# artiom-matvei/RLAO

Hardware: AMD Instinct MI355X
Metric: AO env-steps/sec (batched loops) (higher is better)
Workload: dtype f32; 1 GPU; 8m / 20x20 Shack-Hartmann, 256 batched envs per GPU, integrator closed loop (BASELINE.json configs[1]); envs_per_gpu=256, envs_total=256, resolution=120, n_valid_act=357, n_signal=632, layers=1, controller=leaky integrator, gain 0.5, noise=photon, parallelism=env-shards x1, all-gather of episode returns

## Files before the change

### rlao_amd/csrc/common.hpp

```cpp
#pragma once
#include <hip/hip_runtime.h>
#include <stdint.h>
#include <stddef.h>

#include <string>
#include <vector>

#include "aoenv.h"

namespace ao {

constexpr int kWave = 64;
constexpr int kMaxLayer = 8;
constexpr int kMtN = 624;
constexpr int kMaxSplits = 16;
constexpr int kMaxModes = 512;

int fail(const char* fmt, ...);
#define AO_HIP(call)                                                                          \
    do {                                                                                      \
        hipError_t e_ = (call);                                                               \
        if (e_ != hipSuccess)                                                                 \
            return ::ao::fail("%s:%d: %s -> %s", __FILE__, __LINE__, #call, hipGetErrorString(e_)); \
    } while (0)
// ... 219 lines not shown
    T* ret;
    T* strehl;
    T* scal;
    T* total;
    T* residual;
    const double* part;
    int n_tiles, n_pupil, telemetry_index;
    int n_act, n_valid_act, do_integrate;
    T leak, gain_from_obs;
    double src_scale;
};
template <typename T>
int launch_recon_finish(const FinishArgs<T>& fa, int n_env, hipStream_t st);
template <typename T>
int launch_sh_tail(const T* frame, const T* wfs_max, const ShConst<T>& sc, T* signal, const T* fac_m,
                   const T* fac_m2c_t, int n_modes, const FinishArgs<T>& fa, int n_env, int R, int n_subap, int n_valid,
                   int max_group, hipStream_t st);
struct DetectorCfg {
    int active;
    int photon_noise, bits, emccd;
    float qe, dark_e, fwc, gain, readout_noise;
    uint32_t seed_lo, seed_hi;
    uint32_t frame_counter;
    uint32_t env_offset;
};

}
#include "poisson_alias.hpp"
namespace ao {

struct StepArgs {
    KArgs<float> k;
    ShConst<float> sc;
    FinishArgs<float> fa;
    float* frame;
    int store_phase, store_frame;
    float* signal;
    float* wfs_max;
    const float* fac_m;
    const float* fac_m2c_t;
    const short* slot_of;
    const float* amp_pupil;
    const float* gxa;
    const float* gya;
    DetectorCfg det;
    PoissonAlias pa;
    const float* ring_x[kMaxLayer];
    int ring_splits[kMaxLayer];
    const int* outer_idx;
    int n_outer;
    float* next_zx[kMaxLayer];
    int next_sx[kMaxLayer], next_sy[kMaxLayer];
    const int* inner_idx;
    int n_inner, zx_ld;
    int n_modes, n_subap, n_valid, n_env;
};
int step_fused_supported(int R, int n_subap, int n_valid, int n_act, int n_modes);
int step_alias_capacity(int n_act);
int launch_env_step(const StepArgs& a, hipStream_t st);

template <typename T>
struct RolloutActionArgs {
    const T* obs;
    T* action;
    const T* fr;
    const T* fl_t;
    const int* act_slot;
    const T* sigma_env;
    T gain, sigma;
    int n_act, n_valid_act, n_filter;
    uint32_t seed_lo, seed_hi, counter, env_offset;
};
constexpr size_t kRolloutLdsMax = 160 * 1024;
size_t rollout_action_lds(int n_valid_act, int n_filter, size_t esz);
template <typename T>
int launch_rollout_action(const RolloutActionArgs<T>& a, int n_env, hipStream_t st);

template <typename T>
struct DisturbArgs {
    const T* coefs;
    T* seen;
    const T* modes_t;
    const double* amp;
    const double* freq;
    const double* phase;
    int n_valid_act, n_modes, n_lines;
    int64_t tau;
};
template <typename T>
int launch_disturb_apply(const DisturbArgs<T>& a, int n_env, hipStream_t st);

template <typename T>
int launch_convert_from_f64(const double* src, T* dst, size_t n, hipStream_t st);

template <typename T> struct cx;
struct FftPlan {
    int n;
    int np;
    int n_fac;
    int fac[12];
    unsigned magic_ns[12];
    unsigned magic_m[12];
};
int make_fft_plan(int n, FftPlan* pl);
template <typename T>
struct PyrArgs {
// ... 50 lines not shown
```

### rlao_amd/csrc/env.hip

```cpp
#include <algorithm>
#include <cmath>
#include <cstdarg>
#include <cstdio>
#include <cstring>
#include <initializer_list>
#include <new>
#include <utility>

#include "common.hpp"
#include "detector.hpp"
#include "disturb.hpp"
#include "policy.hpp"
#include "sh_device.hpp"

namespace ao {

static thread_local std::string g_err;

int fail(const char* fmt, ...) {
    char buf[1024];
    va_list ap;
    va_start(ap, fmt);
    vsnprintf(buf, sizeof(buf), fmt, ap);
    va_end(ap);
    g_err = buf;
    return 1;
}

struct LayerClock {
    double ratio[2] = {0, 0};
    double buff[2] = {0, 0};
};

struct RingAhead { bool valid = false; int sx = 0, sy = 0, buf = 0; };

struct Layer {
    int N = 0, S = 0, nin = 0, nout = 0, K = 0;
    size_t scr_off = 0;
    void* ab = nullptr;
    int* inner_idx = nullptr;
    int* outer_idx = nullptr;
    bool have_ab = false, have_in = false, have_out = false;
    double weight = 0;
    LayerClock clk;
    int org[2] = {0, 0};
    uint32_t* mt_cur = nullptr;
    int* pos_cur = nullptr;
    uint32_t* mt_alt = nullptr;
    int* pos_alt = nullptr;
    int ring_pending = 0;
    const void* ring_src = nullptr;
    RingAhead ahead;
    bool gather_next = false;
    bool minmax_dirty = false;
    int env_rounds = 0;
};

}

using namespace ao;

struct AoEnv {
    AoCfg c{};
    int device = 0;
    size_t esz = 4;
    int R = 0, A = 0, nAct = 0, E = 0, L = 0, nSig = 0, nSub = 0, nVal = 0;
    int p = 0, n = 0, n_pupil = 0;
    Layer layer[kMaxLayer];
    size_t scr_elems = 0;
    int Kmax = 0, noutmax = 0, Smax = 0;
    bool uniform = true;
    int last_zx_layer = 0;
    bool per_env_wind = false;
    EnvClock* env_clk[2] = {nullptr, nullptr};
    int clk_cur = 0;
    int wind_pixels = 1;
    LayerTaps* env_taps = nullptr;
    bool per_env_r0 = false;
    std::vector<double> h_r0;
    double* xi_scale = nullptr;
    const double* sigma() const { return per_env_r0 ? xi_scale : nullptr; }
    bool use_coefs_img = false;
    bool defer_ring = true;
    bool have[AOENV_C_COUNT] = {false};
    double units = 1.0;
    void* screen = nullptr;
    void* minmax = nullptr;
    void* zx_pipe = nullptr;
    const void* last_zx = nullptr;
    bool use_lookahead = true;
    void* zx = nullptr;
    void* xbuf = nullptr;
    void* gx = nullptr;
    void* gy = nullptr;
    void* gxt = nullptr;
    void* modes = nullptr;
    void* dm_opd = nullptr;
    int* act_idx = nullptr;
    uint8_t* pupil = nullptr;
    void* opd_atm = nullptr;
    void* coefs = nullptr;
    void* dm_prev = nullptr;
    void* coefs_seen = nullptr;
    void* step_cmd = nullptr;
    void* cmd() const { return step_cmd ? step_cmd : coefs; }
    struct Disturb {
        bool set = false;
        int M = 0, J = 0;
        int64_t t0 = 0;
        void* modes_t = nullptr;
        double* par = nullptr;
        size_t modes_cap = 0, par_cap = 0;
    } disturb;
    float* dm_rows = nullptr;
    void* coefs_img = nullptr;
    void* phase = nullptr;
    void* scal = nullptr;
    double* part = nullptr;
    int n_tiles = 0;
    void* total = nullptr;
    void* residual = nullptr;
    void* wfs_max = nullptr;
    void* amp = nullptr;
    int* subap_idx = nullptr;
    uint8_t* valid2d = nullptr;
// ... 503 lines not shown
    fa.do_integrate = integrate;
    fa.leak = (T)env->c.leak;
    fa.gain_from_obs = (T)gain;
    fa.src_scale = 6.283185307179586476925286766559 / env->c.src_wavelength;
    return fa;
}

template <typename T>
int recon_product(AoEnv* env, int* splits, hipStream_t st) {
    const int Kp = (env->n_modes + 3) & ~3;
    if (env->n_modes > 0 && env->use_factored_recon && env->fac_m2c && env->tbuf &&
        (size_t)Kp * (env->nSig + env->A) < (size_t)env->A * env->nSig) {
        T* t = env->as<T>(env->tbuf);
        if constexpr (std::is_same<T, float>::value) {
            if (env->use_mfma) {
                const int s1 = gemm_splits(env->E, Kp, env->nSig);
                AO_TRY(launch_gemm_nt_mfma(env->as<float>(env->signal), env->as<float>(env->fac_m), t, env->E, Kp, env->nSig, env->nSig,
                                           env->nSig, s1, st));
                *splits = cdiv(env->A, 64) >= 32 ? 1 : gemm_splits(env->E, env->A, Kp);
                int xs = s1;
                if (s1 > 1 && cdiv(env->A, 64) >= 8) {
                    AO_TRY(launch_sum_slabs(t, (size_t)env->E * Kp, s1, st));
                    xs = 1;
                }
                return launch_gemm_nt_mfma(t, env->as<float>(env->fac_m2c), env->as<float>(env->vbuf), env->E, env->A, Kp, Kp, Kp, *splits,
                                           st, xs, (size_t)env->E * Kp);
            }
        }
        *splits = 1;
        AO_TRY(launch_gemm_nt<T>(env->as<T>(env->signal), env->as<T>(env->fac_m), t, env->E, Kp, env->nSig, env->nSig, env->nSig, Kp, st));
        return launch_gemm_nt<T>(t, env->as<T>(env->fac_m2c), env->as<T>(env->vbuf), env->E, env->A, Kp, Kp, Kp, env->A, st);
    }
    return gemm_dispatch<T>(env, env->as<T>(env->signal), env->as<T>(env->recon), env->as<T>(env->vbuf), env->E, env->A, env->nSig,
                            splits, st);
}

template <typename T>
int run_recon(AoEnv* env, const T* d_action, T* d_obs, T* d_reward, T* d_strehl, int telemetry_index, int integrate,
              double gain, hipStream_t st) {
    int splits = 1;
    {
        AO_PROF(env, GEMM_RECON, st);
        AO_TRY(recon_product<T>(env, &splits, st));
    }
    {
        FinishArgs<T> fa = finish_args<T>(env, d_action, d_obs, d_reward, d_strehl, telemetry_index, integrate, gain, splits);
        AO_PROF(env, RECON_FINISH, st);
        AO_TRY(launch_recon_finish<T>(fa, env->E, st));
    }
    if (integrate) AO_TRY(refresh_dense_dm<T>(env, st));
    return 0;
}

template <typename T>
bool fused_step_ok(const AoEnv*) { return false; }
template <>
bool fused_step_ok<float>(const AoEnv* env) {
    return env->use_fused_step && env->use_fast_wfs && env->use_mfma && env->use_fused_tail && env->c.wfs_type == AOENV_WFS_SH && env->c.dm_separable && env->n_modes > 0 &&
           env->c.max_group == 1 && env->L > 0 && env->uniform && env->c.cam_res == env->R && env->force_path == 0 &&
           step_fused_supported(env->R, env->nSub, env->nVal, env->nAct, env->n_modes) != 0;
}

template <typename T>
void fill_phase_args(AoEnv* env, PhaseArgs& pa, PhaseBuffers<T>& pb, int update_atm, int store_atm, int store_phase) {
    pa = PhaseArgs{};
    pa.n_layer = env->L;
    pa.S = env->layer[0].S;
    pa.foot = (env->layer[0].N / 2 - env->R / 2) + 1;
    pa.update_atm = (update_atm && env->L > 0 && !env->atm_user_defined) ? 1 : 0;
    pa.store_atm = store_atm;
    pa.store_phase = store_phase;
    for (int l = 0; l < env->L; ++l) {
        const Layer& y = env->layer[l];
        pa.S_l[l] = y.S;
        pa.foot_l[l] = (y.N / 2 - env->R / 2) + 1;
        pa.screen[l] = env->screen_ptr(l);
        pa.minmax[l] = env->minmax_ptr(l);
        pa.minmax_dirty[l] = y.minmax_dirty ? 1 : 0;
        LayerTaps& t = pa.taps[l];
        t.oy = y.org[0];
        t.ox = y.org[1];
        taps_from_buff(y.clk.buff, t);
        t.weight = y.weight;
    }
    pa.env_taps = env->per_env_wind ? env->env_taps : nullptr;
    pa.n_env = env->E;
    pb = PhaseBuffers<T>{};
    pb.opd_atm = env->as<T>(env->opd_atm);
    pb.coefs = env->as<T>(env->cmd());
    pb.coefs_img = env->use_coefs_img && env->coefs_img ? env->as<T>(env->coefs_img) : nullptr;
    pb.s1a = env->use_coefs_img && env->c.dm_separable ? env->dm_rows : nullptr;
    pb.dm_opd = env->c.dm_separable ? nullptr : env->as<T>(env->dm_opd);
    pb.gx = env->as<T>(env->gx);
    pb.gy = env->as<T>(env->gy);
    pb.gxt = env->as<T>(env->gxt);
    pb.gxa = env->gxa;
    pb.gya = env->gya;
    pb.ga_stride = env->ga_stride;
    pb.act_idx = env->act_idx;
    pb.pupil = env->pupil;
    pb.phase = env->as<T>(env->phase);
    pb.part = env->part;
    pb.wfs_max = env->as<T>(env->wfs_max);
}

template <typename T>
int run_fused_step(AoEnv*, int, const void*, void*, void*, void*, double, bool, hipStream_t) { return fail("fused step: float32 only"); }
template <>
int run_fused_step<float>(AoEnv* env, int i, const void* d_action, void* d_obs, void* d_reward, void* d_strehl, double gain,
                          bool observable, hipStream_t st) {
    if (env->amp_pupil_dirty) {
        const size_t R2 = (size_t)env->R * env->R;
        if (env->h_pupil.size() != R2 || env->h_amp.size() != R2) return fail("pupil / WFS amplitude have not been uploaded");
        std::vector<float> t(R2);
        for (size_t q = 0; q < R2; ++q) t[q] = env->h_pupil[q] ? (float)env->h_amp[q] : -1.f;
        AO_HIP(hipMemcpyAsync(env->amp_pupil, t.data(), R2 * sizeof(float), hipMemcpyHostToDevice, st));
        AO_HIP(hipStreamSynchronize(st));
        env->amp_pupil_dirty = false;
    }
    StepArgs a{};
    PhaseArgs pa;
    PhaseBuffers<float> pb;
    fill_phase_args<float>(env, pa, pb, 1, env->store_opd_atm ? 1 : 0, 1);
    a.k = make_phase_kargs<float>(pa, pb, env->R, env->nAct, env->A, env->c.atm_wavelength, env->c.src_wavelength);
    a.sc = sh_const<float>(env);
    a.fa = finish_args<float>(env, static_cast<const float*>(d_action), static_cast<float*>(d_obs),
                              static_cast<float*>(d_reward), static_cast<float*>(d_strehl), i, 1, gain, 1);
    a.fa.n_tiles = 1;
    a.frame = env->as<float>(env->frame);
    a.store_phase = a.store_frame = (observable || env->store_opd_atm) ? 1 : 0;
    a.signal = env->as<float>(env->signal);
    a.wfs_max = env->as<float>(env->wfs_max);
    a.fac_m = env->as<float>(env->fac_m);
    a.fac_m2c_t = env->as<float>(env->fac_m2c_t);
    a.slot_of = env->slot_of;
    a.amp_pupil = env->amp_pupil;
    a.gxa = env->gxa;
    a.gya = env->gya;
    if (env->det.active) env->det.frame_counter += 1;
    a.det = env->det;
    a.pa = env->alias();
    take_rings(env, a);
    const Layer& y0 = env->layer[0];
    a.outer_idx = y0.outer_idx;
    a.n_outer = y0.nout;
    a.inner_idx = y0.inner_idx;
    a.n_inner = y0.nin;
    a.zx_ld = y0.K;
    a.n_modes = env->n_modes;
    a.n_subap = env->nSub;
    a.n_valid = env->nVal;
    a.n_env = env->E;
    {
        AO_PROF(env, ENV_STEP, st);
        AO_TRY(launch_env_step(a, st));
    }
    rings_written(env);
    return 0;
}

struct SeenCommand {
    AoEnv* env;
    ~SeenCommand() { env->step_cmd = nullptr; }
};
template <typename T>
int apply_disturbance(AoEnv* env, int i, hipStream_t st) {
    const AoEnv::Disturb& d = env->disturb;
    const size_t n = (size_t)env->E * d.M * d.J;
    DisturbArgs<T> a{};
    a.coefs = env->as<T>(env->coefs);
    a.seen = env->as<T>(env->coefs_seen);
    a.modes_t = env->as<T>(d.modes_t);
    a.amp = d.par;
    a.freq = d.par + n;
    a.phase = d.par + 2 * n;
    a.n_valid_act = env->A;
    a.n_modes = d.M;
    a.n_lines = d.J;
    a.tau = d.t0 + (int64_t)i + 1;
    AO_TRY(launch_disturb_apply<T>(a, env->E, st));
    env->step_cmd = env->coefs_seen;
    return refresh_dense_dm<T>(env, st);
}

template <typename T>
int step_t(AoEnv* env, int i, const void* d_action, void* d_obs, void* d_frame, void* d_reward, void* d_strehl,
           double gain, bool observable, hipStream_t st) {
    const bool fused_step = fused_step_ok<T>(env);
    SeenCommand seen{env};
    if (env->disturb.set) AO_TRY(apply_disturbance<T>(env, i, st));
    AO_TRY(advance_atmosphere<T>(env, fused_step, st));
    env->atm_user_defined = false;
    if (fused_step) {
        AO_TRY(run_fused_step<T>(env, i, d_action, d_obs, d_reward, d_strehl, gain, observable, st));
        env->step_cmd = nullptr;
        if (d_frame)
            AO_HIP(hipMemcpyAsync(d_frame, env->frame, (size_t)env->E * env->c.cam_res * env->c.cam_res * sizeof(T),
                                  hipMemcpyDeviceToDevice, st));
        return 0;
// ... 30 lines not shown
        AO_TRY(run_recon<T>(env, static_cast<const T*>(d_action), static_cast<T*>(d_obs), static_cast<T*>(d_reward),
                            static_cast<T*>(d_strehl), i, 1, gain, st));
    }
    if (d_frame)
        AO_HIP(hipMemcpyAsync(d_frame, env->frame, (size_t)env->E * env->c.cam_res * env->c.cam_res * sizeof(T),
                              hipMemcpyDeviceToDevice, st));
    return 0;
}

struct BufInfo {
    void* ptr;
    size_t bytes;
};

int buf_info(AoEnv* env, int which, BufInfo* b) {
    const size_t z = env->esz, E = env->E, R2 = (size_t)env->R * env->R;
    switch (which) {
        case AOENV_B_SCREEN: *b = {nullptr, env->scr_elems * z}; return 0;
        case AOENV_B_OPD_ATM: *b = {env->opd_atm, E * R2 * z}; return 0;
        case AOENV_B_COEFS: *b = {env->coefs, E * env->A * z}; return 0;
        case AOENV_B_PHASE: *b = {env->phase, E * R2 * z}; return 0;
        case AOENV_B_FRAME: *b = {env->frame, E * (size_t)env->c.cam_res * env->c.cam_res * z}; return 0;
        case AOENV_B_SIGNAL: *b = {env->signal, E * env->nSig * z}; return 0;
        case AOENV_B_TOTAL: *b = {env->total, (size_t)env->c.n_loop * E * z}; return 0;
        case AOENV_B_RESIDUAL: *b = {env->residual, (size_t)env->c.n_loop * E * z}; return 0;
        case AOENV_B_WFS_MAX: *b = {env->wfs_max, E * z}; return 0;
        case AOENV_B_XI: *b = {env->last_zx ? const_cast<void*>(env->last_zx) : env->zx, E * env->layer[env->last_zx_layer].K * z}; return 0;
        case AOENV_B_MT_STATE: *b = {nullptr, (size_t)env->L * E * (kMtN + 1) * 4}; return 0;
        case AOENV_B_COUNTERS: *b = {nullptr, 16}; return 0;
        case AOENV_B_DM_PREV: *b = {env->dm_prev, E * env->A * z}; return 0;
        case AOENV_B_COEFS_SEEN: *b = {env->coefs_seen, E * env->A * z}; return 0;
        default: return fail("unknown buffer id %d", which);
    }
}

}

struct DeviceGuard {
    int prev = -1;
    bool ok = false;
    explicit DeviceGuard(int device) {
        if (hipGetDevice(&prev) != hipSuccess) prev = -1;
        ok = prev == device || hipSetDevice(device) == hipSuccess;
        if (prev == device) prev = -1;
    }
    ~DeviceGuard() { if (prev >= 0) (void)hipSetDevice(prev); }
    DeviceGuard(const DeviceGuard&) = delete;
    DeviceGuard& operator=(const DeviceGuard&) = delete;
};
#define AO_CHECK_ENV(env)                                                             \
    if (!(env)) return fail("null AoEnv");                                            \
    DeviceGuard ao_device_guard((env)->device);                                       \
    if (!ao_device_guard.ok) return fail("hipSetDevice(%d) failed", (env)->device)
static int upload_layer_table(AoEnv* env, int kind, int l, const void* h, size_t bytes) {
    if (l < 0 || l >= env->L) return fail("layer %d outside [0, %d)", l, env->L);
    Layer& y = env->layer[l];
    const int S = y.S, N = y.N;
    auto need = [&](size_t n) { return bytes == n ? 0 : fail("ring table %d of layer %d: got %zu bytes, expected %zu", kind, l, bytes, n); };
    if (kind == AOENV_C_AB) {
        AO_TRY(need((size_t)y.nout * y.K * 8));
        for (int j = 0; j < env->L; ++j) forget_lookahead(env->layer[j]);
        AO_TRY(upload_real(env, y.ab, static_cast<const double*>(h), (size_t)y.nout * y.K));
        y.have_ab = true;
        return 0;
    }
    if (kind != AOENV_C_INNER_IDX && kind != AOENV_C_OUTER_IDX) return fail("table %d is not a per-layer table", kind);
    const int cnt = kind == AOENV_C_INNER_IDX ? y.nin : y.nout;
    AO_TRY(need((size_t)cnt * 4));
    const int32_t* ix = static_cast<const int32_t*>(h);
    for (int i = 0; i < cnt; ++i)
        if (ix[i] < 0 || ix[i] >= S * S) return fail("ring index %d out of the %dx%d screen", ix[i], S, S);
    if (kind == AOENV_C_INNER_IDX)
        for (int i = 0; i < cnt; ++i) {
            const int r = ix[i] / S, c = ix[i] % S;
            if (r < 1 || r > N || c < 1 || c > N) return fail("inner ring index %d is not interior", ix[i]);
        }
    AO_HIP(hipMemcpy(kind == AOENV_C_INNER_IDX ? y.inner_idx : y.outer_idx, h, (size_t)cnt * 4, hipMemcpyHostToDevice));
    (kind == AOENV_C_INNER_IDX ? y.have_in : y.have_out) = true;
    return 0;
}

template <typename T>
int atm_update_t(AoEnv* env, hipStream_t st) {
    AO_TRY(advance_atmosphere<T>(env, false, st));
    env->atm_user_defined = false;
    return run_phase<T>(env, 1, 1, st);
}

#define AO_DISPATCH(env, fn, ...) ((env)->c.dtype == AOENV_F32 ? fn<float>(__VA_ARGS__) : fn<double>(__VA_ARGS__))

extern "C" {

const char* aoenv_last_error(void) { return g_err.c_str(); }
int aoenv_abi_version(void) { return AOENV_ABI_VERSION; }

int aoenv_create(const AoCfg* cfg, int device, AoEnv** out) {
    if (!cfg || !out) return fail("aoenv_create: null argument");
    if (cfg->abi_version != AOENV_ABI_VERSION) return fail("ABI version %d != %d", cfg->abi_version, AOENV_ABI_VERSION);
    if (cfg->dtype != AOENV_F32 && cfg->dtype != AOENV_F64) return fail("bad dtype %d", cfg->dtype);
    if (cfg->n_env < 1 || cfg->resolution < 2) return fail("bad n_env / resolution");
    if (cfg->n_layer < 0 || cfg->n_layer > kMaxLayer) return fail("n_layer %d out of range [0, %d]", cfg->n_layer, kMaxLayer);
    if (cfg->n_subap < 1 || cfg->resolution % cfg->n_subap) return fail("resolution %% n_subap != 0");
    if (cfg->n_layer > 0) {
        if (cfg->layer_res < cfg->resolution + 4) return fail("layer_res %d < R + 4", cfg->layer_res);
        if (cfg->n_inner != 8 * cfg->layer_res - 16 || cfg->n_outer != 4 * cfg->layer_res + 4)
            return fail("n_inner / n_outer do not match layer_res");
        for (int l = 0; l < cfg->n_layer; ++l)
            if (cfg->layer_res_l[l] != 0 && cfg->layer_res_l[l] < cfg->resolution + 4)
                return fail("layer_res_l[%d] = %d < R + 4", l, cfg->layer_res_l[l]);
    }
    if (cfg->n_signal != 2 * cfg->n_valid_subap) return fail("n_signal != 2 n_valid_subap");
    if (cfg->wfs_type != AOENV_WFS_SH && cfg->wfs_type != AOENV_WFS_PYRAMID) return fail("unknown wfs_type %d", cfg->wfs_type);
    if (cfg->wfs_type == AOENV_WFS_PYRAMID) {
        if (cfg->pyr_n_res < cfg->resolution || cfg->pyr_n_res % 2 || cfg->cam_res < 1 || cfg->pyr_n_res % cfg->cam_res)
            return fail("pyramid: nRes %d must be even, >= R and a multiple of the camera size %d", cfg->pyr_n_res, cfg->cam_res);
        if (cfg->pyr_n_theta < 1) return fail("pyramid: n_theta must be >= 1");
        if (cfg->pyr_q_lo < 0 || cfg->pyr_q_hi + cfg->n_subap > cfg->cam_res) return fail("pyramid: quadrants outside the camera");
    }
    if (cfg->max_group < 1) return fail("max_group must be >= 1");
    int ndev = 0;
    AO_HIP(hipGetDeviceCount(&ndev));
    if (device < 0 || device >= ndev) return fail("device %d not in [0, %d)", device, ndev);
    DeviceGuard ao_device_guard(device);
    if (!ao_device_guard.ok) return fail("hipSetDevice(%d) failed", device);

    AoEnv* e = new (std::nothrow) AoEnv();
    if (!e) return fail("out of host memory");
    e->c = *cfg;
    e->device = device;
    e->esz = cfg->dtype == AOENV_F32 ? 4 : 8;
    e->R = cfg->resolution; e->A = cfg->n_valid_act; e->nAct = cfg->n_act; e->E = cfg->n_env; e->L = cfg->n_layer;
    e->nSig = cfg->n_signal; e->nSub = cfg->n_subap; e->nVal = cfg->n_valid_subap;
    e->p = e->R / e->nSub; e->n = 2 * e->p;
    e->layer[0].N = cfg->layer_res;
    e->layer[0].S = cfg->layer_res + 2;
    for (int l = 0; l < e->L; ++l) {
        Layer& y = e->layer[l];
        y.N = cfg->layer_res_l[l] ? cfg->layer_res_l[l] : cfg->layer_res;
        y.S = y.N + 2;
        y.nin = 8 * y.N - 16;
        y.nout = 4 * y.N + 4;
        y.K = y.nin + y.nout;
        y.scr_off = e->scr_elems;
        e->scr_elems += (size_t)e->E * y.S * y.S;
        e->Kmax = std::max(e->Kmax, y.K);
        e->noutmax = std::max(e->noutmax, y.nout);
        e->Smax = std::max(e->Smax, y.S);
        if (y.N != e->layer[0].N) e->uniform = false;
    }
    const size_t z = e->esz, E = e->E, R2 = (size_t)e->R * e->R;
    int rc = 0;
    auto A_ = [&](void** p, size_t bytes) { if (!rc) rc = dmalloc(e, p, bytes); };
    if (e->L > 0) {
        A_(&e->screen, e->scr_elems * z);
        A_(&e->minmax, (size_t)e->L * E * 2 * z);
        if (cfg->dtype == AOENV_F32) {
            A_(&e->zx_pipe, (size_t)2 * e->L * E * e->Kmax * z);
        }
        A_(&e->zx, E * e->Kmax * z);
        A_(&e->xbuf, (size_t)e->L * kMaxSplits * E * e->noutmax * z);
        for (int l = 0; l < e->L; ++l) {
            Layer& y = e->layer[l];
            A_((void**)&y.mt_cur, E * kMtN * 4);
            A_((void**)&y.pos_cur, E * 4);
            A_((void**)&y.mt_alt, E * kMtN * 4);
            A_((void**)&y.pos_alt, E * 4);
            if (l > 0 && e->uniform) {
                y.ab = e->layer[0].ab;
                y.inner_idx = e->layer[0].inner_idx;
                y.outer_idx = e->layer[0].outer_idx;
                continue;
            }
            A_(&y.ab, (size_t)y.nout * y.K * z);
            A_((void**)&y.inner_idx, (size_t)y.nin * 4);
            A_((void**)&y.outer_idx, (size_t)y.nout * 4);
        }
    }
    A_(&e->gx, (size_t)e->R * e->nAct * z);
    A_(&e->gy, (size_t)e->R * e->nAct * z);
    A_(&e->gxt, (size_t)((e->nAct + 3) & ~3) * (size_t)(cdiv(e->R, 128) * 128) * z);
    if (!cfg->dm_separable) {
        A_(&e->modes, R2 * e->A * z);
        A_(&e->dm_opd, E * R2 * z);
    }
    A_((void**)&e->act_idx, (size_t)e->A * 4);
    A_((void**)&e->pupil, R2);
    A_(&e->opd_atm, E * R2 * z);
    A_(&e->coefs, E * e->A * z);
    A_(&e->coefs_seen, E * e->A * z);
    A_(&e->dm_prev, E * e->A * z);
    A_(&e->phase, E * R2 * z);
    A_(&e->scal, E * 4 * z);
    e->n_tiles = phase_tiles(e->R, e->nAct, e->esz);
    A_((void**)&e->part, E * (size_t)e->n_tiles * 4 * sizeof(double));
    A_(&e->total, (size_t)cfg->n_loop * E * z);
    A_(&e->residual, (size_t)cfg->n_loop * E * z);
    A_(&e->wfs_max, E * z);
    A_(&e->amp, R2 * z);
    A_((void**)&e->subap_idx, (size_t)e->nVal * 4);
    A_((void**)&e->valid2d, (size_t)e->nSub * e->nSub);
    A_((void**)&e->slot_of, (size_t)e->nSub * e->nSub * sizeof(short));
    A_((void**)&e->amp_pupil, R2 * sizeof(float));
    e->ga_stride = std::max(8, ((cdiv(e->nAct, 4) + 3) / 4) * 4);
    A_((void**)&e->gxa, (size_t)(cdiv(e->R, 128) * 128) * 4 * e->ga_stride * sizeof(float));
    A_((void**)&e->gya, (size_t)(cdiv(e->R, 128) * 128) * 4 * e->ga_stride * sizeof(float));
    if (e->A > 1024 && !rc) { rc = alloc_dm_rows(e); e->use_coefs_img = true; }
    A_(&e->sh_ref, (size_t)2 * e->nVal * z);
    A_(&e->tw, (size_t)e->n * 2 * z);
    A_(&e->phs, (size_t)e->p * 2 * z);
    A_(&e->frame, E * (size_t)cfg->cam_res * cfg->cam_res * z);
    A_(&e->signal, E * e->nSig * z);
    A_(&e->recon, (size_t)e->A * e->nSig * z);
    A_(&e->fac_m, (size_t)kMaxModes * e->nSig * z);
    A_(&e->fac_m2c_t, (size_t)kMaxModes * e->A * z);
    if (cfg->wfs_type == AOENV_WFS_PYRAMID) {
        const size_t N = cfg->pyr_n_res;
        e->pyr_chunk = cfg->pyr_n_theta < 4 ? cfg->pyr_n_theta : 4;
        A_(&e->pyr_mask, N * N * 2 * z);
        A_(&e->pyr_tt, (size_t)cfg->pyr_n_theta * R2 * z);
        A_(&e->pyr_tw, N * 2 * z);
        A_(&e->pyr_t1, E * e->pyr_chunk * (size_t)e->R * N * 2 * z);
        A_(&e->pyr_t2, E * e->pyr_chunk * N * N * 2 * z);
    }
    A_(&e->vbuf, (size_t)kMaxSplits * E * e->A * z);
    {
        const PoissonAliasHost& ph = poisson_alias_host();
        int budget = (int)ph.tab.size();
        if (cfg->wfs_type == AOENV_WFS_SH && e->p == fast6::P && e->R <= 128 && e->nAct <= 32) budget = std::min(budget, step_alias_capacity(e->nAct));
        ph.prefix(budget, &e->alias_words, &e->alias_lmax);
// ... 1390 lines not shown
```

### rlao_amd/csrc/step_kernel.hip

```cpp
#include "common.hpp"

#include "sh_device.hpp"
#include "detector.hpp"
#include "ring_device.hpp"

#include "camera_sh6.hpp"


namespace ao {

typedef float f32x4s __attribute__((ext_vector_type(4)));

template <typename P>
__device__ inline float ld_or0(const P* __restrict__ p, long idx, bool ok) {
    const float v = (float)p[ok ? idx : 0];
    return ok ? v : 0.f;
}

namespace fstep {
constexpr int TX = 128, PR = 64;
constexpr int WR = 16 + 3, WC = 32 + 4;
constexpr int WC4 = WC / 4;
constexpr int NV4 = (WR * WC4 + 63) / 64;
}

struct StepLds {
    int cimg, s1, mapt, slot, e0, sl, img, total;
    int tab, tab_cap;
};

static StepLds step_lds_layout(int n_act, int n_subap, int n_valid, int n_modes) {
    using namespace fstep;
    StepLds L;
    const int nAp = (n_act + 3) & ~3, SS = nAp + 1;
    int o = 0;
    auto take = [&](int words) { const int at = o; o += (words + 3) & ~3; return at; };
    const int sl_words = (2 * n_valid + 3) & ~3, img_words = n_act * n_act + n_modes;
    L.cimg = take(n_act * n_act);
    L.s1 = take(2 * PR * SS);
    L.mapt = take(16 * WR * WC);
    L.tab = L.cimg;
    L.tab_cap = o - L.tab;
    L.slot = take((n_subap * n_subap + 1) / 2);
    L.e0 = take(std::max(2 * n_valid * fast6::EST, sl_words + img_words));
    L.sl = L.e0;
    L.img = L.e0 + sl_words;
    L.total = o;
    return L;
}

template <bool PE>
__device__ inline const LayerTaps& step_taps(const PhaseArgs& pa, int l, int e) {
    if constexpr (PE) return pa.env_taps[(size_t)l * pa.n_env + e];
    else return pa.taps[l];
}

template <int KS, bool PE>
__global__ void __launch_bounds__(1024) k_env_step_sh6(const StepArgs a, const StepLds L) {
    using namespace fstep;
    using fast6::EST;
    extern __shared__ __align__(16) unsigned char lds_raw[];
    float* lds = reinterpret_cast<float*>(lds_raw);
    const KArgs<float>& k = a.k;
    const int R = k.R, nA = k.n_act, S = k.pa.S;
    const int nAp = (nA + 3) & ~3, SS = nAp + 1;
    float* cimg = lds + L.cimg;
    float* s1 = lds + L.s1;
    const int w_ = threadIdx.x >> 6;
    float* mapt = lds + L.mapt + w_ * (WR * WC);
    short* slot_s = reinterpret_cast<short*>(lds + L.slot);
    cplx<float>* E0 = reinterpret_cast<cplx<float>*>(lds + L.e0);
    float* sl = lds + L.sl;
    float* img_s = lds + L.img;
    const uint32_t* tab_s = reinterpret_cast<const uint32_t*>(lds + L.tab);
    __shared__ double red[4][16];
    __shared__ double red_tail[16];
    __shared__ float red_mx[16];

    const int e = blockIdx.x;
    const int tid = threadIdx.x, w = tid >> 6, lane = tid & 63;
    const int lc = lane & 15, lq = lane >> 4;
    const int band = w >> 2, cg = w & 3;
    const size_t pix0 = (size_t)e * R * R;
    const int n_sub = a.n_subap, n_valid = a.n_valid;

    const float ctab = fast6::cos_table_lane<float>();
    f32x4s gx_raw[2][2], gy_raw[2];
#pragma unroll
    for (int tt = 0; tt < 2; ++tt) {
        const f32x4s* src = reinterpret_cast<const f32x4s*>(a.gxa) + (2 * cg + tt) * 2 * 64 + (tid & 63);
        gx_raw[tt][0] = src[0];
        gx_raw[tt][1] = src[64];
    }
    const int rt = w >> 1, ct = w & 1;
    {
        const f32x4s* src = reinterpret_cast<const f32x4s*>(a.gya) + rt * 2 * 64 + (tid & 63);
        gy_raw[0] = src[0];
        gy_raw[1] = src[64];
    }
    float mm_pre[kMaxLayer];
#pragma unroll
    for (int l = 0; l < kMaxLayer; ++l)
        mm_pre[l] = l < k.pa.n_layer ? static_cast<const float*>(k.pa.minmax[l])[2 * e + (tid & 1)] : 0.f;
    const bool has_act = tid < k.n_valid_act;
    const int act_px = k.pb.act_idx[has_act ? tid : 0];
    const float act_c = k.pb.coefs[(size_t)e * k.n_valid_act + (has_act ? tid : 0)];
    const short slot_v = a.slot_of[tid < n_sub * n_sub ? tid : 0];
    for (int i = tid; i < nA * nA; i += 1024) cimg[i] = 0.f;
    for (int i = tid; i < 2 * PR * SS; i += 1024) s1[i] = 0.f;
    if (tid < n_sub * n_sub) slot_s[tid] = slot_v;
    for (int i = tid + 1024; i < n_sub * n_sub; i += 1024) slot_s[i] = a.slot_of[i];
    lds_barrier();
    if (has_act) cimg[act_px] = act_c;
    float breg[2][KS];
#pragma unroll
    for (int tt = 0; tt < 2; ++tt) {
        const float t[8] = {gx_raw[tt][0][0], gx_raw[tt][0][1], gx_raw[tt][0][2], gx_raw[tt][0][3],
                            gx_raw[tt][1][0], gx_raw[tt][1][1], gx_raw[tt][1][2], gx_raw[tt][1][3]};
#pragma unroll
        for (int ks = 0; ks < KS; ++ks) breg[tt][ks] = t[ks];
    }

    lds_barrier();
    {
        const int ix = 16 * ct + lc;
        float av[KS], bv[KS];
        {
            const float t[8] = {gy_raw[0][0], gy_raw[0][1], gy_raw[0][2], gy_raw[0][3], gy_raw[1][0], gy_raw[1][1], gy_raw[1][2], gy_raw[1][3]};
#pragma unroll
            for (int ks = 0; ks < KS; ++ks) av[ks] = t[ks];
        }
#pragma unroll
        for (int ks = 0; ks < KS; ++ks) {
            const int iy = lq + 4 * ks;
            bv[ks] = ld_or0(cimg, iy * nA + ix, iy < nA && ix < nA);
        }
        f32x4s d = {0.f, 0.f, 0.f, 0.f};
#pragma unroll
        for (int ks = 0; ks < KS; ++ks) d = __builtin_amdgcn_mfma_f32_16x16x4f32(av[ks], bv[ks], d, 0, 0, 0);
        if (ix < nA) {
#pragma unroll
            for (int r = 0; r < 4; ++r) s1[(16 * rt + 4 * lq + r) * SS + ix] = d[r];
        }
    }

    {
        bool any = false;
        for (int l = 0; l < k.pa.n_layer; ++l) {
            const float* x = a.ring_x[l];
            if (x == nullptr) continue;
            any = true;
            const LayerTaps& tl = step_taps<PE>(k.pa, l, e);
            if (PE && !tl.ring) continue;
            float* map = const_cast<float*>(static_cast<const float*>(k.pa.screen[l])) + (size_t)e * S * S;
            const size_t slab = (size_t)a.n_env * a.n_outer;
            const int oy = tl.oy, ox = tl.ox;
            for (int q = tid; q < a.n_outer; q += 1024) {
                float xv[kMaxSplits];
#pragma unroll
                for (int z = 0; z < kMaxSplits; ++z)
                    xv[z] = x[(size_t)(z < a.ring_splits[l] ? z : 0) * slab + (size_t)e * a.n_outer + q];
                float v = xv[0];
#pragma unroll
                for (int z = 1; z < kMaxSplits; ++z) v += z < a.ring_splits[l] ? xv[z] : 0.f;
                const int idx = a.outer_idx[q];
                int pr = idx / S + oy, pc = idx % S + ox;
                pr = pr >= S ? pr - S : pr;
                pc = pc >= S ? pc - S : pc;
                map[pr * S + pc] = v;
            }
        }
        if (any) __syncthreads();
        if (!PE) {
            for (int l = 0; l < k.pa.n_layer; ++l)
                if (a.next_zx[l] != nullptr)
                    gather_ring<float>(static_cast<const float*>(k.pa.screen[l]), a.next_zx[l], a.inner_idx, S, a.n_inner, a.zx_ld,
                                       a.next_sx[l], a.next_sy[l], k.pa.taps[l].oy, k.pa.taps[l].ox, e, tid, 1024);
        }
    }

    __shared__ float lohi[kMaxLayer][2];
    __shared__ float red_lo[16], red_hi[16];
    for (int l = 0; l < k.pa.n_layer; ++l) {
        float* mm = const_cast<float*>(static_cast<const float*>(k.pa.minmax[l])) + 2 * e;
        const bool dirty = k.pa.minmax_dirty[l] || (PE && a.ring_x[l] != nullptr && step_taps<PE>(k.pa, l, e).ring);
        if (!dirty) {
            float pre = 0.f;
#pragma unroll
            for (int q = 0; q < kMaxLayer; ++q) pre = q == l ? mm_pre[q] : pre;
            if (tid < 2) lohi[l][tid] = pre;
            continue;
        }
        const float* map = static_cast<const float*>(k.pa.screen[l]) + (size_t)e * S * S;
        const int n4 = (S * S) / 4;
        float lo = 3.0e38f, hi = -3.0e38f;
        if ((S * S) % 4 == 0) {
            for (int i0 = tid; i0 < n4; i0 += 4 * 1024) {
                f32x4s v[4];
#pragma unroll
                for (int u = 0; u < 4; ++u) v[u] = *reinterpret_cast<const f32x4s*>(map + 4 * (i0 + 1024 * u < n4 ? i0 + 1024 * u : i0));
#pragma unroll
                for (int u = 0; u < 4; ++u)
#pragma unroll
                    for (int d = 0; d < 4; ++d) { lo = v[u][d] < lo ? v[u][d] : lo; hi = v[u][d] > hi ? v[u][d] : hi; }
            }
        } else {
            for (int i = tid; i < S * S; i += 1024) { const float v = map[i]; lo = v < lo ? v : lo; hi = v > hi ? v : hi; }
        }
        for (int off = 32; off > 0; off >>= 1) {
            const float ol = __shfl_down(lo, off), oh = __shfl_down(hi, off);
            lo = ol < lo ? ol : lo;
            hi = oh > hi ? oh : hi;
        }
        lds_barrier();
        if (lane == 0) { red_lo[w] = lo; red_hi[w] = hi; }
        lds_barrier();
        if (tid == 0) {
            for (int i = 1; i < 16; ++i) { lo = red_lo[i] < lo ? red_lo[i] : lo; hi = red_hi[i] > hi ? red_hi[i] : hi; }
            lohi[l][0] = lo; lohi[l][1] = hi;
            mm[0] = lo; mm[1] = hi;
        }
    }

    double s_atm = 0.0, q_atm = 0.0, s_res = 0.0, q_res = 0.0;
    for (int pass = 0; pass < (R + PR - 1) / PR; ++pass) {
        const int y0 = pass * PR;
        const int tye = min(PR, R - y0);
        const int yl = 16 * band + lc, y = y0 + yl;
        const bool row_ok = yl < tye;
        if (pass == 0) lds_barrier();
        f32x4s apv[2];
#pragma unroll
        for (int tt = 0; tt < 2; ++tt) {
            const int x = 16 * (2 * cg + tt) + 4 * lq;
            const bool okp = row_ok && x < R;
            apv[tt] = *reinterpret_cast<const f32x4s*>(a.amp_pupil + (okp ? (size_t)y * R + x : 0));
            if (!okp) apv[tt] = f32x4s{-1.f, -1.f, -1.f, -1.f};
        }
// ... 146 lines not shown
        if (!ok) {
#pragma unroll
            for (int u = 0; u < 6; ++u) Ia[u] = Ib[u] = 0.f;
        }
    }
    if (ok) {
        const int kk = a.sc.subap_idx[s];
        li = kk / n_sub;
        lj = kk - li * n_sub;
    }
    if (a.det.active) {
        f32x16s pxv = camera_pack(Ia, Ib);
        if (cam_photons) {
            asm volatile("s_waitcnt vmcnt(0)" ::: "memory");
            lds_barrier();
        }
        camera_sh6_lane(pxv, ok, (uint32_t)((li * 6) * R + lj * 6 + q3), R, (uint32_t)e, a.det, tab_s, a.pa.lmax);
        camera_unpack(pxv, Ia, Ib);
    }
    if (ok) {
        if (a.store_frame) {
            float* fr = a.frame + pix0 + (size_t)(li * 6) * R + lj * 6 + q3;
#pragma unroll
            for (int u = 0; u < 6; ++u) {
                fr[(size_t)u * R] = Ia[u];
                fr[(size_t)u * R + 3] = Ib[u];
            }
        }
#pragma unroll
        for (int u = 0; u < 6; ++u) {
            mx = Ia[u] > mx ? Ia[u] : mx;
            mx = Ib[u] > mx ? Ib[u] : mx;
        }
    }
    if (a.store_frame && a.det.active && (a.det.dark_e > 0.f || a.det.readout_noise != 0.f)) {
        const float rtab = recip_table_lane();
        for (int idx = tid; idx < n_sub * n_sub * 9; idx += 1024) {
            const int kk = idx / 9, j = idx - 9 * kk;
            if (slot_s[kk] < 0) {
                const int i2 = kk / n_sub, j2 = kk - i2 * n_sub;
                uint32_t pix[4];
                sh6_quad_pixels(j, i2 * 6, j2 * 6, R, pix);
                f32x4d v = {0.f, 0.f, 0.f, 0.f};
                detector_quad<false>(v, pix, pix[0], (uint32_t)e, a.det, rtab, a.pa);
#pragma unroll
                for (int s4 = 0; s4 < 4; ++s4) a.frame[pix0 + pix[s4]] = v[s4];
            }
        }
    }
    int late0;
    asm volatile("v_mov_b32 %0, 0" : "=v"(late0) : "v"(mx));
    const int n_sig = 2 * n_valid, n4 = n_sig / 4, A = k.n_valid_act;
    const int km = tid >> 4, l16 = tid & 15;
    f32x4s mv[10];
    if (4 * w < a.n_modes) {
        const f32x4s* row = reinterpret_cast<const f32x4s*>(a.fac_m + (size_t)(km < a.n_modes ? km : 0) * n_sig);
#pragma unroll
        for (int j = 0; j < 10; ++j) mv[j] = row[(l16 + 16 * j < n4 ? l16 + 16 * j : 0) + late0];
    } else {
#pragma unroll
        for (int j = 0; j < 10; ++j) mv[j] = f32x4s{0.f, 0.f, 0.f, 0.f};
    }
    const float ref0 = a.sc.ref[ok ? s : 0], ref1 = a.sc.ref[ok ? n_valid + s : 0];
    float act_prev = 0.f, dm_prev_c = 0.f;
    if (a.fa.do_integrate) {
        const size_t io = (size_t)e * (nA * nA) + (has_act ? act_px : 0) + late0;
        act_prev = (a.fa.gain_from_obs != 0.f) ? a.fa.obs[io] : a.fa.action[io];
        dm_prev_c = a.fa.dm_prev[(size_t)e * k.n_valid_act + (has_act ? tid : 0) + late0];
    }
    for (int off = 32; off > 0; off >>= 1) {
        const float o = __shfl_down(mx, off);
        mx = o > mx ? o : mx;
    }
    if (lane == 0) red_mx[w] = mx;
    lds_barrier();
    mx = red_mx[0];
#pragma unroll
    for (int q = 1; q < 16; ++q) mx = red_mx[q] > mx ? red_mx[q] : mx;
    if (tid == 0) a.wfs_max[e] = mx;
    for (int i = tid; i < nA * nA; i += 1024) img_s[i] = 0.f;
    const float cut = a.sc.threshold * mx;
    {
        float norm = 0.f, m0 = 0.f, m1 = 0.f;
#pragma unroll
        for (int u = 0; u < 6; ++u) {
            const float xa = Ia[u] < cut ? 0.f : Ia[u], xb = Ib[u] < cut ? 0.f : Ib[u];
            const float rs = xa + xb;
            norm += rs;
            m0 += rs * (float)u;
            m1 += xa * (float)q3 + xb * (float)(q3 + 3);
        }
        norm += __shfl_down(norm, 1) + __shfl_down(norm, 2);
        m0 += __shfl_down(m0, 1) + __shfl_down(m0, 2);
        m1 += __shfl_down(m1, 1) + __shfl_down(m1, 2);
        if (ok && q3 == 0) {
            float c0 = 0.f, c1 = 0.f;
            if (norm != 0.f) {
                c0 = m0 / norm;
                c1 = m1 / norm;
            }
            const float v0 = (c0 - ref0) / a.sc.units, v1 = (c1 - ref1) / a.sc.units;
            sl[s] = v0;
            sl[n_valid + s] = v1;
            a.signal[(size_t)e * 2 * n_valid + s] = v0;
            a.signal[(size_t)e * 2 * n_valid + n_valid + s] = v1;
        }
    }
    lds_barrier();

    const int img = nA * nA;
    float* tm = img_s + img;
    {
        const f32x4s* s4 = reinterpret_cast<const f32x4s*>(sl);
        float acc = 0.f;
#pragma unroll
        for (int j = 0; j < 10; ++j) {
            const bool okj = l16 + 16 * j < n4;
            const f32x4s sv = s4[okj ? l16 + 16 * j : 0];
            const float d = ((mv[j][0] * sv[0] + mv[j][1] * sv[1]) + mv[j][2] * sv[2]) + mv[j][3] * sv[3];
            acc += okj ? d : 0.f;
        }
#pragma unroll
        for (int off = 8; off > 0; off >>= 1) acc += __shfl_xor(acc, off, 16);
        if (km < a.n_modes && l16 == 0) tm[km] = acc;
    }
    const int n_grp = (A + 3) / 4, g = tid >> 2, part = tid & 3;
    const bool g_ok = g < n_grp;
    f32x4s cv[13];
    int late1;
    asm volatile("v_mov_b32 %0, 0" : "=v"(late1) : "v"(late0));
    if (16 * w < n_grp) {
#pragma unroll
        for (int j = 0; j < 13; ++j)
            __builtin_memcpy(&cv[j], a.fac_m2c_t + (part + 4 * j < a.n_modes ? (size_t)(part + 4 * j) * A + 4 * (g_ok ? g : 0) : 0) + late1, 16);
    } else {
#pragma unroll
        for (int j = 0; j < 13; ++j) cv[j] = f32x4s{0.f, 0.f, 0.f, 0.f};
    }
    lds_barrier();
    double ss = 0.0;
    {
        float acc[4] = {0.f, 0.f, 0.f, 0.f};
#pragma unroll
        for (int j = 0; j < 13; ++j) {
            const bool okj = part + 4 * j < a.n_modes;
            const float t = tm[okj ? part + 4 * j : 0];
#pragma unroll
            for (int d = 0; d < 4; ++d) acc[d] += okj ? cv[j][d] * t : 0.f;
        }
#pragma unroll
        for (int d = 0; d < 4; ++d) {
            acc[d] += __shfl_xor(acc[d], 1, 4);
            acc[d] += __shfl_xor(acc[d], 2, 4);
        }
        if (has_act) {
            const float mine = part == 0 ? acc[0] : (part == 1 ? acc[1] : (part == 2 ? acc[2] : acc[3]));
            if (a.fa.do_integrate) {
                const float act = (a.fa.gain_from_obs != 0.f) ? a.fa.gain_from_obs * act_prev : act_prev;
                const float cn = dm_prev_c * a.fa.leak + act * 1e-6f;
                a.fa.coefs[(size_t)e * A + tid] = cn;
                a.fa.dm_prev[(size_t)e * A + tid] = cn;
            }
            const float o = -mine * 1e6f;
            img_s[act_px] = o;
            ss += (double)o * (double)o;
        }
    }
    lds_barrier();
    {
        float* ob = a.fa.obs + (size_t)e * img;
        for (int q = tid; q < img; q += 1024) ob[q] = img_s[q];
    }
    ss = wave_sum_f64(ss);
    if (lane == 0) red_tail[w] = ss;
    lds_barrier();
    if (tid == 0) {
        double tot = 0;
        for (int q = 0; q < 16; ++q) tot += red_tail[q];
        if (a.fa.reward) a.fa.reward[e] = (float)(-sqrt(tot));
        if (a.fa.ret && a.fa.do_integrate) a.fa.ret[e] += (float)(-sqrt(tot));
    }
}

int step_fused_supported(int R, int n_subap, int n_valid, int n_act, int n_modes) {
    if (R % n_subap || R / n_subap != fast6::P) return 0;
    if (R > fstep::TX || R % 4) return 0;
    if (n_valid > 16 * 21 || n_subap * n_subap > 32767 || n_act > 32) return 0;
    if (n_modes < 1 || n_modes > 52 || (2 * n_valid) % 4 != 0 || 2 * n_valid > 640) return 0;
    const StepLds L = step_lds_layout(n_act, n_subap, n_valid, n_modes);
    return (size_t)L.total * 4 <= 160 * 1024 - 1024 ? 1 : 0;
}

int step_alias_capacity(int n_act) { return step_lds_layout(n_act, 1, 1, 1).tab_cap; }

int launch_env_step(const StepArgs& a, hipStream_t st) {
    const StepLds L = step_lds_layout(a.k.n_act, a.n_subap, a.n_valid, a.n_modes);
    if (a.det.active && a.det.photon_noise && (!a.pa.tab || a.pa.words > L.tab_cap || a.pa.lmax < palias::kCoarseStep))
        return fail("fused step: the photon-noise tables are missing or do not fit (%d words, room for %d)", a.pa.words, L.tab_cap);
    const size_t lds = (size_t)L.total * 4;
    const int v = a.k.n_act <= 24 ? 0 : 1;
    const bool pe = a.k.pa.env_taps != nullptr;
    const void* fn = v == 0 ? (pe ? reinterpret_cast<const void*>(k_env_step_sh6<6, true>) : reinterpret_cast<const void*>(k_env_step_sh6<6, false>))
                            : (pe ? reinterpret_cast<const void*>(k_env_step_sh6<8, true>) : reinterpret_cast<const void*>(k_env_step_sh6<8, false>));
    static size_t attr_set[4] = {0, 0, 0, 0};
    const int vi = 2 * v + (pe ? 1 : 0);
    if (lds > 64 * 1024 && lds > attr_set[vi]) {
        AO_HIP(hipFuncSetAttribute(fn, hipFuncAttributeMaxDynamicSharedMemorySize, (int)lds));
        attr_set[vi] = lds;
    }
    if (v == 0 && !pe) hipLaunchKernelGGL((k_env_step_sh6<6, false>), dim3(a.n_env), dim3(1024), lds, st, a, L);
    else if (v == 0) hipLaunchKernelGGL((k_env_step_sh6<6, true>), dim3(a.n_env), dim3(1024), lds, st, a, L);
    else if (!pe) hipLaunchKernelGGL((k_env_step_sh6<8, false>), dim3(a.n_env), dim3(1024), lds, st, a, L);
    else hipLaunchKernelGGL((k_env_step_sh6<8, true>), dim3(a.n_env), dim3(1024), lds, st, a, L);
    AO_HIP(hipGetLastError());
    return 0;
}

}
```

Baseline: 5.512 million env-steps/s.

## Fuse ring write, zx gather and min/max into a single crossing pass

Moves the atmosphere ring update to the top of the fused step kernel. Each thread now writes its ring value, feeds the next-step zx gather through a precomputed ring-to-zx slot table, and computes the screen min/max in registers during the same pass. This removes the __syncthreads and the separate gather_ring and min/max sweeps over the screen. The host builds and validates the slot table, and the fused path is gated on it being valid. The change also introduces a late-bound wave index and adds more host-side setup and register pressure.

```diff
diff --git a/rlao_amd/csrc/common.hpp b/rlao_amd/csrc/common.hpp
--- a/rlao_amd/csrc/common.hpp
+++ b/rlao_amd/csrc/common.hpp
@@ -295,6 +295,7 @@
     float* next_zx[kMaxLayer];
     int next_sx[kMaxLayer], next_sy[kMaxLayer];
     const int* inner_idx;
+    const int* ring_to_zx;
     int n_inner, zx_ld;
     int n_modes, n_subap, n_valid, n_env;
 };
diff --git a/rlao_amd/csrc/env.hip b/rlao_amd/csrc/env.hip
--- a/rlao_amd/csrc/env.hip
+++ b/rlao_amd/csrc/env.hip
@@ -10,6 +10,7 @@
 #include "common.hpp"
 #include "detector.hpp"
 #include "disturb.hpp"
+#include "ring_slots.hpp"
 #include "policy.hpp"
 #include "sh_device.hpp"
 
@@ -71,6 +72,9 @@
     int Kmax = 0, noutmax = 0, Smax = 0;
     bool uniform = true;
     int last_zx_layer = 0;
+    std::vector<int32_t> h_inner, h_outer;
+    int* ring_to_zx = nullptr;
+    bool ring_slots_ok = false;
     bool per_env_wind = false;
     EnvClock* env_clk[2] = {nullptr, nullptr};
     int clk_cur = 0;
@@ -680,13 +684,20 @@
     return 0;
 }
 
+static bool crossing_head_ok(const AoEnv* env) {
+    const Layer& y = env->layer[0];
+    const int foot = (y.N / 2 - env->R / 2) + 1;
+    return foot >= 3 && foot + env->R + 3 <= y.S && y.nout <= 1024 && y.nin <= 1024 && y.S * y.S <= 16 * 1024 && (y.S * y.S) % 4 == 0 &&
+           env->ring_slots_ok;
+}
+
 template <typename T>
 bool fused_step_ok(const AoEnv*) { return false; }
 template <>
 bool fused_step_ok<float>(const AoEnv* env) {
     return env->use_fused_step && env->use_fast_wfs && env->use_mfma && env->use_fused_tail && env->c.wfs_type == AOENV_WFS_SH && env->c.dm_separable && env->n_modes > 0 &&
            env->c.max_group == 1 && env->L > 0 && env->uniform && env->c.cam_res == env->R && env->force_path == 0 &&
-           step_fused_supported(env->R, env->nSub, env->nVal, env->nAct, env->n_modes) != 0;
+           step_fused_supported(env->R, env->nSub, env->nVal, env->nAct, env->n_modes) != 0 && crossing_head_ok(env);
 }
 
 template <typename T>
@@ -773,6 +784,7 @@
     a.outer_idx = y0.outer_idx;
     a.n_outer = y0.nout;
     a.inner_idx = y0.inner_idx;
+    a.ring_to_zx = env->ring_to_zx;
     a.n_inner = y0.nin;
     a.zx_ld = y0.K;
     a.n_modes = env->n_modes;
@@ -909,6 +921,17 @@
     if (!(env)) return fail("null AoEnv");                                            \
     DeviceGuard ao_device_guard((env)->device);                                       \
     if (!ao_device_guard.ok) return fail("hipSetDevice(%d) failed", (env)->device)
+static int build_ring_slots(AoEnv* env) {
+    const Layer& y = env->layer[0];
+    env->ring_slots_ok = false;
+    if ((int)env->h_inner.size() != y.nin || (int)env->h_outer.size() != y.nout || !env->ring_to_zx) return 0;
+    std::vector<int32_t> where((size_t)y.S * y.S), tab((size_t)kRingDirs * y.nout);
+    if (!build_ring_to_zx(env->h_inner.data(), y.nin, env->h_outer.data(), y.nout, y.S, where.data(), tab.data())) return 0;
+    AO_HIP(hipMemcpy(env->ring_to_zx, tab.data(), tab.size() * 4, hipMemcpyHostToDevice));
+    env->ring_slots_ok = true;
+    return 0;
+}
+
 static int upload_layer_table(AoEnv* env, int kind, int l, const void* h, size_t bytes) {
     if (l < 0 || l >= env->L) return fail("layer %d outside [0, %d)", l, env->L);
     Layer& y = env->layer[l];
@@ -934,6 +957,10 @@
         }
     AO_HIP(hipMemcpy(kind == AOENV_C_INNER_IDX ? y.inner_idx : y.outer_idx, h, (size_t)cnt * 4, hipMemcpyHostToDevice));
     (kind == AOENV_C_INNER_IDX ? y.have_in : y.have_out) = true;
+    if (l == 0 || env->uniform) {
+        (kind == AOENV_C_INNER_IDX ? env->h_inner : env->h_outer).assign(ix, ix + cnt);
+        AO_TRY(build_ring_slots(env));
+    }
     return 0;
 }
 
@@ -1032,6 +1059,7 @@
             A_((void**)&y.inner_idx, (size_t)y.nin * 4);
             A_((void**)&y.outer_idx, (size_t)y.nout * 4);
         }
+        A_((void**)&e->ring_to_zx, (size_t)kRingDirs * e->layer[0].nout * 4);
     }
     A_(&e->gx, (size_t)e->R * e->nAct * z);
     A_(&e->gy, (size_t)e->R * e->nAct * z);
diff --git a/rlao_amd/csrc/ring_slots.hpp b/rlao_amd/csrc/ring_slots.hpp
--- /dev/null
+++ b/rlao_amd/csrc/ring_slots.hpp
@@ -0,0 +1,52 @@
+#pragma once
+#include <stdint.h>
+
+#if defined(__HIPCC__) || defined(__CUDACC__)
+#define AO_RING_HD __host__ __device__
+#else
+#define AO_RING_HD
+#endif
+
+namespace ao {
+
+constexpr int kRingDirs = 9;
+
+AO_RING_HD inline int ring_dir(int sx, int sy) { return 3 * (sy + 1) + (sx + 1); }
+
+AO_RING_HD inline bool ring_source_on_ring(int idx, int S, int sx, int sy) {
+    const int r = idx / S - sy, c = idx % S - sx;
+    return r == 0 || r == S - 1 || c == 0 || c == S - 1;
+}
+
+inline bool build_ring_to_zx(const int32_t* inner_idx, int n_inner, const int32_t* outer_idx, int n_outer, int S, int32_t* where,
+                             int32_t* table) {
+    if (S < 3 || n_outer != 4 * S - 4) return false;
+    for (int i = 0; i < S * S; ++i) where[i] = -1;
+    for (int q = 0; q < n_outer; ++q) {
+        const int idx = outer_idx[q];
+        if (idx < 0 || idx >= S * S) return false;
+        const int r = idx / S, c = idx % S;
+        if (!(r == 0 || r == S - 1 || c == 0 || c == S - 1) || where[idx] >= 0) return false;
+        where[idx] = q;
+    }
+    for (int k = 0; k < n_inner; ++k) {
+        const int idx = inner_idx[k];
+        if (idx < 0 || idx >= S * S) return false;
+        const int r = idx / S, c = idx % S;
+        if (r < 1 || r > S - 2 || c < 1 || c > S - 2) return false;
+    }
+    for (int sy = -1; sy <= 1; ++sy)
+        for (int sx = -1; sx <= 1; ++sx) {
+            int32_t* t = table + (size_t)ring_dir(sx, sy) * n_outer;
+            for (int q = 0; q < n_outer; ++q) t[q] = -1;
+            for (int k = 0; k < n_inner; ++k) {
+                if (!ring_source_on_ring(inner_idx[k], S, sx, sy)) continue;
+                const int src = (inner_idx[k] / S - sy) * S + (inner_idx[k] % S - sx);
+                if (t[where[src]] >= 0) return false;
+                t[where[src]] = k;
+            }
+        }
+    return true;
+}
+
+}
diff --git a/rlao_amd/csrc/step_kernel.hip b/rlao_amd/csrc/step_kernel.hip
--- a/rlao_amd/csrc/step_kernel.hip
+++ b/rlao_amd/csrc/step_kernel.hip
@@ -3,6 +3,7 @@
 #include "sh_device.hpp"
 #include "detector.hpp"
 #include "ring_device.hpp"
+#include "ring_slots.hpp"
 
 #include "camera_sh6.hpp"
 
@@ -85,19 +86,6 @@
     const int n_sub = a.n_subap, n_valid = a.n_valid;
 
     const float ctab = fast6::cos_table_lane<float>();
-    f32x4s gx_raw[2][2], gy_raw[2];
-#pragma unroll
-    for (int tt = 0; tt < 2; ++tt) {
-        const f32x4s* src = reinterpret_cast<const f32x4s*>(a.gxa) + (2 * cg + tt) * 2 * 64 + (tid & 63);
-        gx_raw[tt][0] = src[0];
-        gx_raw[tt][1] = src[64];
-    }
-    const int rt = w >> 1, ct = w & 1;
-    {
-        const f32x4s* src = reinterpret_cast<const f32x4s*>(a.gya) + rt * 2 * 64 + (tid & 63);
-        gy_raw[0] = src[0];
-        gy_raw[1] = src[64];
-    }
     float mm_pre[kMaxLayer];
 #pragma unroll
     for (int l = 0; l < kMaxLayer; ++l)
@@ -106,6 +94,87 @@
     const int act_px = k.pb.act_idx[has_act ? tid : 0];
     const float act_c = k.pb.coefs[(size_t)e * k.n_valid_act + (has_act ? tid : 0)];
     const short slot_v = a.slot_of[tid < n_sub * n_sub ? tid : 0];
+
+    float* ring_red = lds + L.mapt;
+    for (int l = 0; l < k.pa.n_layer; ++l) {
+        const float* x = a.ring_x[l];
+        if (x == nullptr) continue;
+        const LayerTaps& tl = step_taps<PE>(k.pa, l, e);
+        if (PE && !tl.ring) continue;
+        float* map = const_cast<float*>(static_cast<const float*>(k.pa.screen[l])) + (size_t)e * S * S;
+        const size_t slab = (size_t)a.n_env * a.n_outer;
+        const int oy = tl.oy, ox = tl.ox;
+        const bool has_q = tid < a.n_outer;
+        const int q = has_q ? tid : 0;
+        float xv[kMaxSplits];
+#pragma unroll
+        for (int z = 0; z < kMaxSplits; ++z)
+            xv[z] = x[(size_t)(z < a.ring_splits[l] ? z : 0) * slab + (size_t)e * a.n_outer + q];
+        const int idx = a.outer_idx[q];
+        float* nz = PE ? nullptr : a.next_zx[l];
+        const int sx = a.next_sx[l], sy = a.next_sy[l];
+        const bool has_k = tid < a.n_inner;
+        int zslot = -1, zidx = 0;
+        if (nz != nullptr) {
+            zslot = a.ring_to_zx[ring_dir(sx, sy) * a.n_outer + q];
+            zidx = a.inner_idx[has_k ? tid : 0];
+        }
+        const int n4 = (S * S) / 4;
+        f32x4s sv[4];
+#pragma unroll
+        for (int u = 0; u < 4; ++u) sv[u] = *reinterpret_cast<const f32x4s*>(map + 4 * (tid + 1024 * u < n4 ? tid + 1024 * u : 0));
+        const bool z_old = nz != nullptr && has_k && !ring_source_on_ring(zidx, S, sx, sy);
+        float zv = 0.f;
+        if (nz != nullptr) zv = map[z_old ? torus(zidx / S - sy, zidx % S - sx, oy, ox, S) : 0];
+
+        float v = xv[0];
+#pragma unroll
+        for (int z = 1; z < kMaxSplits; ++z) v += z < a.ring_splits[l] ? xv[z] : 0.f;
+        float lo = 3.0e38f, hi = -3.0e38f;
+        if (has_q) {
+            map[torus(idx / S, idx % S, oy, ox, S)] = v;
+            if (zslot >= 0) nz[(size_t)e * a.zx_ld + zslot] = v;
+            lo = hi = v;
+        }
+        const int ra = oy, rb = oy == 0 ? S - 1 : oy - 1, ca = ox, cb = ox == 0 ? S - 1 : ox - 1;
+        const float rS = 1.f / (float)S;
+#pragma unroll
+        for (int u = 0; u < 4; ++u) {
+            const int at = 4 * (tid + 1024 * u);
+            int pr = (int)(((float)at + 0.5f) * rS), pc = at - pr * S;
+            if (pc < 0) { pr -= 1; pc += S; }
+            if (pc >= S) { pr += 1; pc -= S; }
+#pragma unroll
+            for (int d = 0; d < 4; ++d) {
+                const bool wrap = pc + d >= S;
+                const int r = wrap ? pr + 1 : pr, c = wrap ? pc + d - S : pc + d;
+                const bool skip = tid + 1024 * u >= n4 || r == ra || r == rb || c == ca || c == cb;
+                lo = !skip && sv[u][d] < lo ? sv[u][d] : lo;
+                hi = !skip && sv[u][d] > hi ? sv[u][d] : hi;
+            }
+        }
+        for (int off = 32; off > 0; off >>= 1) {
+            const float ol = __shfl_down(lo, off), oh = __shfl_down(hi, off);
+            lo = ol < lo ? ol : lo;
+            hi = oh > hi ? oh : hi;
+        }
+        if (lane == 0) { ring_red[32 * l + w] = lo; ring_red[32 * l + 16 + w] = hi; }
+        if (z_old) nz[(size_t)e * a.zx_ld + tid] = zv;
+    }
+
+    f32x4s gx_raw[2][2], gy_raw[2];
+#pragma unroll
+    for (int tt = 0; tt < 2; ++tt) {
+        const f32x4s* src = reinterpret_cast<const f32x4s*>(a.gxa) + (2 * cg + tt) * 2 * 64 + (tid & 63);
+        gx_raw[tt][0] = src[0];
+        gx_raw[tt][1] = src[64];
+    }
+    const int rt = w >> 1, ct = w & 1;
+    {
+        const f32x4s* src = reinterpret_cast<const f32x4s*>(a.gya) + rt * 2 * 64 + (tid & 63);
+        gy_raw[0] = src[0];
+        gy_raw[1] = src[64];
+    }
     for (int i = tid; i < nA * nA; i += 1024) cimg[i] = 0.f;
     for (int i = tid; i < 2 * PR * SS; i += 1024) s1[i] = 0.f;
     if (tid < n_sub * n_sub) slot_s[tid] = slot_v;
@@ -144,46 +213,23 @@
         }
     }
 
-    {
-        bool any = false;
-        for (int l = 0; l < k.pa.n_layer; ++l) {
-            const float* x = a.ring_x[l];
-            if (x == nullptr) continue;
-            any = true;
-            const LayerTaps& tl = step_taps<PE>(k.pa, l, e);
-            if (PE && !tl.ring) continue;
-            float* map = const_cast<float*>(static_cast<const float*>(k.pa.screen[l])) + (size_t)e * S * S;
-            const size_t slab = (size_t)a.n_env * a.n_outer;
-            const int oy = tl.oy, ox = tl.ox;
-            for (int q = tid; q < a.n_outer; q += 1024) {
-                float xv[kMaxSplits];
-#pragma unroll
-                for (int z = 0; z < kMaxSplits; ++z)
-                    xv[z] = x[(size_t)(z < a.ring_splits[l] ? z : 0) * slab + (size_t)e * a.n_outer + q];
-                float v = xv[0];
-#pragma unroll
-                for (int z = 1; z < kMaxSplits; ++z) v += z < a.ring_splits[l] ? xv[z] : 0.f;
-                const int idx = a.outer_idx[q];
-                int pr = idx / S + oy, pc = idx % S + ox;
-                pr = pr >= S ? pr - S : pr;
-                pc = pc >= S ? pc - S : pc;
-                map[pr * S + pc] = v;
-            }
-        }
-        if (any) __syncthreads();
-        if (!PE) {
-            for (int l = 0; l < k.pa.n_layer; ++l)
-                if (a.next_zx[l] != nullptr)
-                    gather_ring<float>(static_cast<const float*>(k.pa.screen[l]), a.next_zx[l], a.inner_idx, S, a.n_inner, a.zx_ld,
-                                       a.next_sx[l], a.next_sy[l], k.pa.taps[l].oy, k.pa.taps[l].ox, e, tid, 1024);
-        }
-    }
-
     __shared__ float lohi[kMaxLayer][2];
     __shared__ float red_lo[16], red_hi[16];
     for (int l = 0; l < k.pa.n_layer; ++l) {
         float* mm = const_cast<float*>(static_cast<const float*>(k.pa.minmax[l])) + 2 * e;
-        const bool dirty = k.pa.minmax_dirty[l] || (PE && a.ring_x[l] != nullptr && step_taps<PE>(k.pa, l, e).ring);
+        if (a.ring_x[l] != nullptr && (!PE || step_taps<PE>(k.pa, l, e).ring)) {
+            if (tid == 0) {
+                float lo = ring_red[32 * l], hi = ring_red[32 * l + 16];
+                for (int i = 1; i < 16; ++i) {
+                    lo = ring_red[32 * l + i] < lo ? ring_red[32 * l + i] : lo;
+                    hi = ring_red[32 * l + 16 + i] > hi ? ring_red[32 * l + 16 + i] : hi;
+                }
+                lohi[l][0] = lo; lohi[l][1] = hi;
+                mm[0] = lo; mm[1] = hi;
+            }
+            continue;
+        }
+        const bool dirty = k.pa.minmax_dirty[l] != 0;
         if (!dirty) {
             float pre = 0.f;
 #pragma unroll
@@ -436,8 +482,9 @@
     asm volatile("v_mov_b32 %0, 0" : "=v"(late0) : "v"(mx));
     const int n_sig = 2 * n_valid, n4 = n_sig / 4, A = k.n_valid_act;
     const int km = tid >> 4, l16 = tid & 15;
+    const int wl = (tid + late0) >> 6;
     f32x4s mv[10];
-    if (4 * w < a.n_modes) {
+    if (4 * wl < a.n_modes) {
         const f32x4s* row = reinterpret_cast<const f32x4s*>(a.fac_m + (size_t)(km < a.n_modes ? km : 0) * n_sig);
 #pragma unroll
         for (int j = 0; j < 10; ++j) mv[j] = row[(l16 + 16 * j < n4 ? l16 + 16 * j : 0) + late0];
@@ -456,7 +503,7 @@
         const float o = __shfl_down(mx, off);
         mx = o > mx ? o : mx;
     }
-    if (lane == 0) red_mx[w] = mx;
+    if (lane == 0) red_mx[wl] = mx;
     lds_barrier();
     mx = red_mx[0];
 #pragma unroll
@@ -513,7 +560,7 @@
     f32x4s cv[13];
     int late1;
     asm volatile("v_mov_b32 %0, 0" : "=v"(late1) : "v"(late0));
-    if (16 * w < n_grp) {
+    if (16 * wl < n_grp) {
 #pragma unroll
         for (int j = 0; j < 13; ++j)
             __builtin_memcpy(&cv[j], a.fac_m2c_t + (part + 4 * j < a.n_modes ? (size_t)(part + 4 * j) * A + 4 * (g_ok ? g : 0) : 0) + late1, 16);
@@ -556,7 +603,7 @@
         for (int q = tid; q < img; q += 1024) ob[q] = img_s[q];
     }
     ss = wave_sum_f64(ss);
-    if (lane == 0) red_tail[w] = ss;
+    if (lane == 0) red_tail[wl] = ss;
     lds_barrier();
     if (tid == 0) {
         double tot = 0;
```

Result: no change. 5.505 million env-steps/s (-0.1%).
